# Intsights/PySubstringSearch

Measured on AMD Instinct MI355X. Metric: queries/sec (batched) + index-build GB/s on 512MB chunk, 1/2/4/8 GPU, higher is better.
Workload: dtype u64

## Files before the change

### pysubstringsearch_amd/csrc/msd_sort.hip

```cpp
#include "msd_sort.h"

#include <algorithm>
#include <type_traits>
#include <vector>

#include "prims.h"
#include "scan.h"
#include "text_keys.h"

namespace pss {

constexpr int MSD_D = 10;
constexpr u32 MSD_BINS = 1u << MSD_D;
constexpr int MSD_BLOCK = 512;
constexpr int MSD_WAVES = MSD_BLOCK / kWave;
constexpr int MSD_IPT = 16;
constexpr u32 MSD_TILE = MSD_BLOCK * MSD_IPT;
constexpr u32 MSD_WIN = 6144;
#ifndef PSS_LS_WINDOW
#define PSS_LS_WINDOW 8
#endif
constexpr u32 MSD_TILE_CAP = 8184 - PSS_LS_WINDOW;
constexpr u32 MSD_MAX_BUCKET = 4088;
constexpr int MSD_TAG_BITS = MSD_D + 1;
constexpr u32 MSD_TAG_SPAN = 1u << MSD_TAG_BITS;
constexpr int MSD_RAW_TAG_BITS = 6;
constexpr u32 MSD_RAW_TAG_SPAN = 1u << MSD_RAW_TAG_BITS;
constexpr u32 MSD_G1_RANGES = 1024;
constexpr u32 MSD_G2_RANGE = 16 * MSD_TILE;

struct MsdRange {
    u32 seg, start, end;
};

struct MsdTile2 {
    u32 start, count, d_last;
};

struct MsdArgs {
    const u8 *codes;
    int code_bits, key_chars, plus_one, key_drop;
    u32 n;
    int key_bits;
    int idx_bits;
    u32 tiles_per_range1, num_ranges1;
    u32 *T;
    u32 *J1;
    u32 *J;
    MsdRange *ranges2;
    u32 *seg_first;
    u32 *counters;
    const u64 *dense;
    const u64 *in;
    u64 *out;
    int lsd;
    u32 *T2;
    const u32 *Jb;
    const struct MsdTile2 *tiles2;
    u32 *status;
    const u8 *raw;
    const u8 *lut;
    u8 *codes_out;
    u32 *bad;
};

__device__ __forceinline__ void keep_load(u64 &v) { asm volatile("" : "+v"(v)); }
__device__ __forceinline__ void keep_load(uint4 &v) { asm volatile("" : "+v"(v.x), "+v"(v.y), "+v"(v.z), "+v"(v.w)); }

__device__ __forceinline__ void lds_barrier()
{
    asm volatile("s_waitcnt lgkmcnt(0)\n\ts_barrier" ::: "memory");
}


template <bool FROM_TEXT>
__device__ __forceinline__ void msd_load_tile(const MsdArgs &a, u32 base, u32 valid, u64 (&elem)[MSD_IPT], u32 (&dig)[MSD_IPT],
                                              int shift2)
{
    const u32 tid = threadIdx.x;
    if (FROM_TEXT) {
        const u32 i0 = base + tid * MSD_IPT;
        u64 key[MSD_IPT] = {};
        if (i0 < a.n) text_keys16(a.codes, i0, a.code_bits, a.key_chars, a.plus_one, a.key_drop, a.n, key);
        const int rest_bits = a.key_bits - MSD_D;
        const u64 rest_mask = (1ull << rest_bits) - 1ull;
#pragma unroll
        for (int r = 0; r < MSD_IPT; ++r) {
            dig[r] = (u32)(key[r] >> rest_bits) & (MSD_BINS - 1u);
            elem[r] = ((key[r] & rest_mask) << a.idx_bits) | (u64)(i0 + r);
        }
    } else {
#pragma unroll
        for (int r = 0; r < MSD_IPT; ++r) {
            const u32 p = r * MSD_BLOCK + tid;
            elem[r] = p < valid ? a.in[base + p] : 0ull;
            dig[r] = (u32)(elem[r] >> shift2) & (MSD_BINS - 1u);
        }
    }
}

template <bool FROM_TEXT>
__device__ __forceinline__ bool msd_valid(u32 base, u32 valid, int r, u32 n)
{
    const u32 tid = threadIdx.x;
    (void)base;
    (void)n;
    return FROM_TEXT ? (tid * MSD_IPT + r < valid) : (r * MSD_BLOCK + tid < valid);
}

template <bool FROM_TEXT>
__global__ __launch_bounds__(MSD_BLOCK) void msd_hist_kernel(MsdArgs a)
{
    __shared__ u32 hist[MSD_BINS];
    __shared__ u32 histb[FROM_TEXT ? MSD_BINS : 1];
    const u32 tid = threadIdx.x, r = blockIdx.x;
    u32 e0, e1;
    if (FROM_TEXT) {
        if (r >= a.num_ranges1) return;
        e0 = r * a.tiles_per_range1 * MSD_TILE;
        const u64 end = (u64)(r + 1) * a.tiles_per_range1 * MSD_TILE;
        e1 = end < a.n ? (u32)end : a.n;
    } else {
        if (r >= a.counters[0]) return;
        e0 = a.ranges2[r].start;
        e1 = a.ranges2[r].end;
    }
    for (u32 i = tid; i < MSD_BINS; i += MSD_BLOCK) {
        hist[i] = 0;
        if (FROM_TEXT) histb[i] = 0;
    }
    __syncthreads();
    const int shift2 = a.idx_bits + a.key_bits - 2 * MSD_D;
    if (FROM_TEXT) {
        const int b = a.code_bits;
        const int top = a.lsd ? 2 * MSD_D : MSD_D;
        const int m = (top + b - 1) / b;
        const u32 wmask = (m * b >= 32) ? ~0u : ((1u << (m * b)) - 1u);
        const int down = m * b - top;
        uint4 nlo = make_uint4(0, 0, 0, 0), nhi = nlo;
        if (e0 + tid * MSD_IPT < e1) {
            const uint4 *p = reinterpret_cast<const uint4 *>(a.codes + e0 + tid * MSD_IPT);
// ... 412 lines not shown
            if (lp[k] != 0xffffffffu) lp[k] = (lp[k] & 0xffffu) + (u32)s_start[lp[k] >> 22];
#pragma unroll
        for (int h = 0; h < MSD_PIECES2; ++h) {
            if (h * MSD_TILE >= valid) break;
            if (h) __syncthreads();
#pragma unroll
            for (int k = 0; k < IPT; ++k) {
                const u32 q = lp[k] - h * MSD_TILE;
                if (q < MSD_TILE) exch[q] = elem[k];
            }
            if (FROM_TEXT && h == MSD_PIECES2 - 1 && (u64)base + MSD_TILE2 < e1) load_ahead(base + MSD_TILE2);
            lds_barrier();
#pragma unroll
            for (int k = 0; k < (int)(MSD_TILE / BLOCK); ++k) {
                const u32 q = k * BLOCK + tid, p = h * MSD_TILE + q;
                if (p < valid) {
                    u64 e = exch[q];
                    u32 d;
                    if (FROM_TEXT) {
                        d = (u32)(e >> 14) & (MSD_BINS - 1u);
                        e = ((e >> 24) << a.idx_bits) | (u64)(base + ((u32)e & (MSD_TILE2 - 1u)));
                    } else {
                        d = (u32)(e >> shift2) & (MSD_BINS - 1u);
                        e = (e & low_mask2) | ((u64)(hist[d] >> 16) << shift2);
                    }
                    a.out[s_delta[d] + p] = e;
                }
            }
        }
    }
}

constexpr u32 LB_A = 1u << 30, LB_P = 2u << 30, LB_STATE = 3u << 30, LB_VALUE = LB_A - 1u;
constexpr int LB_WINDOW = 4;

struct LbAsk {
    u32 v[LB_WINDOW];
};
__device__ __forceinline__ void lb_ask(const u32 *status, u32 p, LbAsk &q)
{
#pragma unroll
    for (u32 w = 0; w < (u32)LB_WINDOW; ++w) {
        const u32 r = p > w ? p - 1 - w : 0u;
        q.v[w] = __hip_atomic_load(&status[(size_t)r * MSD_BINS + threadIdx.x], __ATOMIC_RELAXED, __HIP_MEMORY_SCOPE_AGENT);
    }
}
__device__ __forceinline__ void lb_begin(u32 *status, u32 t, u32 c, LbAsk &q)
{
    if (t == 0) return;
    __hip_atomic_store(&status[(size_t)t * MSD_BINS + threadIdx.x], LB_A | c, __ATOMIC_RELAXED, __HIP_MEMORY_SCOPE_AGENT);
    lb_ask(status, t, q);
}
__device__ __forceinline__ u32 lb_finish(u32 *status, u32 t, u32 c, u32 first, LbAsk &q)
{
    u32 off = first;
    if (t != 0) {
        u32 sum = 0, p = t;
        for (;;) {
            const u32 p0 = p;
            bool stop = false, done = false;
#pragma unroll
            for (u32 w = 0; w < (u32)LB_WINDOW; ++w) {
                if (!stop && w < p0) {
                    const u32 st = q.v[w] & LB_STATE;
                    if (st == 0) {
                        stop = true;
                    } else {
                        sum += q.v[w] & LB_VALUE;
                        --p;
                        if (st == LB_P) done = stop = true;
                    }
                }
            }
            if (done || p == 0) break;
            lb_ask(status, p, q);
        }
        off = sum;
    }
    __hip_atomic_store(&status[(size_t)t * MSD_BINS + threadIdx.x], LB_P | (off + c), __ATOMIC_RELAXED, __HIP_MEMORY_SCOPE_AGENT);
    return off;
}


__global__ __launch_bounds__(MSD_BINS) void msd_tiles2_kernel(const u32 *J1, MsdTile2 *tiles, u32 *counters)
{
    __shared__ u32 scr[MSD_BINS / kWave + 1];
    const u32 d = threadIdx.x;
    const u32 s = J1[d], e = J1[d + 1];
    const u32 nr = (e - s + MSD_TILE2 - 1) / MSD_TILE2;
    u32 total = 0, D = 0;
    const u32 first = block_excl_sum<MSD_BINS / kWave>(nr, scr, &total);
    const u32 dn = block_excl_sum<MSD_BINS / kWave>(nr ? 1u : 0u, scr, &D);
    if (d == 0) counters[0] = total + (MSD_BINS - D);
    if (nr == 0) {
        const u32 dd = D + (d - dn);
        tiles[total + (d - dn)] = MsdTile2{s, 0u, dd | 0x80000000u};
    }
    for (u32 k = 0; k < nr; ++k) {
        const u32 ts = s + k * MSD_TILE2;
        tiles[first + k] = MsdTile2{ts, min(MSD_TILE2, e - ts), dn | (k + 1 == nr ? 0x80000000u : 0u)};
    }
}

__global__ __launch_bounds__(1024) void msd_scatter_lb_kernel(MsdArgs a)
{
    constexpr int BLOCK = 1024;
    constexpr int IPT = MSD_TILE2 / BLOCK;
    __shared__ __attribute__((aligned(16))) u64 exch[MSD_TILE];
    __shared__ u32 hist[MSD_BINS], s_delta[MSD_BINS];
    __shared__ u16 s_start[MSD_BINS];
    __shared__ u32 scr[BLOCK / kWave + 1];
    __shared__ u32 s_ticket;
    const u32 tid = threadIdx.x;
    const u32 nt = a.counters[0];
    const int shift2 = a.idx_bits + a.key_bits - 2 * MSD_D;
    const u64 low_mask2 = (1ull << shift2) - 1ull;
    hist[tid] = 0;
    __syncthreads();
    for (;;) {
        if (tid == 0) s_ticket = atomicAdd(&a.counters[8], 1u);
        __syncthreads();
        const u32 t = s_ticket;
        if (t >= nt) break;
        const MsdTile2 td = a.tiles2[t];
        const u32 base = td.start, valid = td.count;
        u64 elem[IPT];
        u32 lp[IPT];
#pragma unroll
        for (int k = 0; k < IPT; ++k) {
            const u32 p = k * BLOCK + tid;
            elem[k] = p < valid ? a.in[base + p] : 0ull;
        }
#pragma unroll
        for (int k = 0; k < IPT; ++k) {
            const u32 p = k * BLOCK + tid;
            const u32 d = (u32)(elem[k] >> shift2) & (MSD_BINS - 1u);
            lp[k] = p < valid ? (atomicAdd(&hist[d], 1u) | (d << 22)) : 0xffffffffu;
        }
        __syncthreads();
        const u32 c = hist[tid];
        LbAsk ask;
        lb_begin(a.status, t, c, ask);
        const u32 ex = block_excl_sum<BLOCK / kWave>(c, scr, nullptr);
        s_start[tid] = (u16)ex;
        hist[tid] = 0;
        __syncthreads();
        const u64 tag = (u64)(td.d_last & (MSD_RAW_TAG_SPAN - 1u)) << shift2;
#pragma unroll
        for (int k = 0; k < IPT; ++k)
            if (lp[k] != 0xffffffffu) lp[k] = (lp[k] & 0xffffu) + (u32)s_start[lp[k] >> 22];
#pragma unroll
        for (int h = 0; h < MSD_PIECES2; ++h) {
            if (h && h * MSD_TILE >= valid) break;
            if (h) __syncthreads();
#pragma unroll
            for (int k = 0; k < IPT; ++k) {
                const u32 q = lp[k] - h * MSD_TILE;
                if (q < MSD_TILE) exch[q] = elem[k];
            }
            if (h == 0) {
                if (t == 0 && tid == 0) a.J[0] = 0;
                const u32 off = lb_finish(a.status, t, c, a.Jb[tid], ask);
                if (td.d_last >> 31) a.J[(size_t)tid * MSD_BINS + (td.d_last & (MSD_BINS - 1u)) + 1u] = off + c;
                s_delta[tid] = off - ex;
            }
            __syncthreads();
#pragma unroll
            for (int k = 0; k < (int)(MSD_TILE / BLOCK); ++k) {
                const u32 q = k * BLOCK + tid, p = h * MSD_TILE + q;
                if (p < valid) {
                    const u64 e = exch[q];
                    const u32 d = (u32)(e >> shift2) & (MSD_BINS - 1u);
                    a.out[s_delta[d] + p] = (e & low_mask2) | tag;
                }
            }
        }
    }
}


struct InNonEmpty {
    const u32 *J;
    __device__ u64 operator()(u64 j) const { return J[j + 1] > J[j] ? 1u : 0u; }
};

__global__ __launch_bounds__(256) void msd_compact_kernel(const u32 *J, u32 nb, const u64 *rank, u32 *cstart, u32 *counters, u32 *cj)
{
    u32 mx = 0;
    for (u32 j = blockIdx.x * blockDim.x + threadIdx.x; j < nb; j += gridDim.x * blockDim.x) {
        const u32 s = J[j], e = J[j + 1];
        if (e > s) {
            cstart[rank[j]] = s;
            if (cj) cj[rank[j]] = j;
            mx = max(mx, e - s);
        }
    }
    mx = wave_incl_max(mx);
    if (lane_id() == kWave - 1 && mx) atomicMax(&counters[1], mx);
}

struct TilePlan {
    u32 win, cap;
    const u32 *cj;
};
__device__ __forceinline__ bool msd_tile_head(const u32 *cstart, u32 ne, u32 n, u32 k, TilePlan tp)
{
    if (tp.cj) {
        if (k == 0 || (tp.cj[k] >> MSD_RAW_TAG_BITS) != (tp.cj[k - 1] >> MSD_RAW_TAG_BITS)) return true;
    } else if ((k & (MSD_TAG_SPAN - 1u)) == 0) {
        return true;
    }
    const u32 w = cstart[k] / tp.win;
    if (cstart[k - 1] / tp.win != w) return true;
    if (k + 1 < ne && cstart[k + 1] / tp.win == w) return false;
    u32 lo = 0, hi = k;
    const u32 ws = w * tp.win;
    while (lo < hi) {
        const u32 mid = (lo + hi) >> 1;
        if (cstart[mid] < ws) lo = mid + 1; else hi = mid;
    }
    const u32 end = k + 1 < ne ? cstart[k + 1] : n;
    return end - cstart[lo] > tp.cap;
}

struct InTileHead {
    const u32 *cstart;
    u32 ne, n;
    TilePlan tp;
    __device__ u64 operator()(u64 k) const { return msd_tile_head(cstart, ne, n, (u32)k, tp) ? 1u : 0u; }
};

struct InTileHeadDev {
    const u32 *cstart;
    const u64 *nep;
    u32 n;
    TilePlan tp;
    __device__ u64 operator()(u64 k) const
    {
        const u32 ne = (u32)*nep;
        return (k < ne && msd_tile_head(cstart, ne, n, (u32)k, tp)) ? 1u : 0u;
    }
};
__global__ __launch_bounds__(256) void msd_tiles_dev_kernel(const u32 *cstart, const u64 *nep, u32 n, const u64 *rank, const u64 *total,
                                                              u32 *tile_first, TilePlan tp)
{
    const u32 ne = (u32)*nep;
    if (blockIdx.x == 0 && threadIdx.x == 0) tile_first[*total] = ne;
    for (u32 k = blockIdx.x * blockDim.x + threadIdx.x; k < ne; k += gridDim.x * blockDim.x) {
        if (msd_tile_head(cstart, ne, n, k, tp)) tile_first[rank[k]] = k;
    }
}

__global__ __launch_bounds__(256) void msd_tiles_kernel(const u32 *cstart, u32 ne, u32 n, const u64 *rank, const u64 *total,
                                                          u32 *tile_first, TilePlan tp)
{
    if (blockIdx.x == 0 && threadIdx.x == 0) tile_first[*total] = ne;
    for (u32 k = blockIdx.x * blockDim.x + threadIdx.x; k < ne; k += gridDim.x * blockDim.x) {
        if (msd_tile_head(cstart, ne, n, k, tp)) tile_first[rank[k]] = k;
    }
// ... 533 lines not shown
            u32 ties = 0;
            ls_rows<LS_GROUP>(rows, [&](auto full, int g) __attribute__((always_inline)) {
                u64 cur[LS_GROUP], prv[LS_GROUP], nxt[LS_GROUP];
#pragma unroll
                for (int j = 0; j < LS_GROUP; ++j) {
                    const int o = (g + j) * MSD_BLOCK;
                    cur[j] = my[o];
                    prv[j] = o == 0 ? exch[tid - (tid != 0 ? 1u : 0u)] : my[o - 1];
                    nxt[j] = my[o + 1];
                }
#pragma unroll
                for (int j = 0; j < LS_GROUP; ++j) {
                    keep_load(cur[j]);
                    keep_load(prv[j]);
                    keep_load(nxt[j]);
                }
#pragma unroll
                for (int j = 0; j < LS_GROUP; ++j) {
                    const int o = (g + j) * MSD_BLOCK;
                    bool tie = (prv[j] ^ cur[j]) < same;
                    if (o == 0) tie = tie && tid != 0;
                    const bool tie_next = (nxt[j] ^ cur[j]) < same && (decltype(full)::value || o + tid + 1u < count);
                    if (decltype(full)::value || o + tid < count) {
                        out[o] = ((u32)cur[j] & imask) | (tie ? flag : 0u);
                        ties |= ((tie || tie_next) ? 1u << (g + j) : 0u) | (tie ? 0x10000u << (g + j) : 0u);
                    }
                }
            });
            if (em != nullptr) {
                u32 *const s_count = &scr[MSD_WAVES + 3];
                for (u32 m = ties & 0xffffu; m != 0; m &= m - 1u) {
                    const u32 r = (u32)__builtin_ctz(m);
                    const u32 p = r * MSD_BLOCK + tid;
                    const u32 slot = e0 + atomicAdd(s_count, 1u);
                    em->st_pos[slot] = e0 + p;
                    em->st_idx[slot] = ((u32)exch[p] & imask) | ((ties >> (16u + r)) << 31);
                }
            }
        }
        prev_t = t;
        prev_ok = !failed;
        if (!more) break;
        t += stride;
        cur = nxt;
        nxt = t + stride < nt ? tiles[t + stride] : MsdTile{0, 0, 0, 0};
    }
    if (em) {
        lds_barrier();
        if (tid == 0 && prev_ok) em->blk_cnt[prev_t] = scr[MSD_WAVES + 3];
    }
}

#include "ss_sort_impl.h"


static size_t msd_max_tiles(uint32_t n)
{
    return (size_t)n / (SS_WIN / 2) + ((size_t)MSD_BINS * MSD_BINS) / MSD_RAW_TAG_SPAN + 8;
}

static size_t msd_max_tiles2(uint32_t n) { return (size_t)n / MSD_TILE2 + MSD_BINS + 8; }

static bool msd_use_lsd(uint32_t n)
{
    const char *e = knob("PSS_MSD_LSD");
    return !(e && atoi(e) == 0) && n < (1u << 30);
}

size_t msd_workspace_bytes(uint32_t n)
{
    const size_t max_ranges2 = (size_t)n / MSD_G2_RANGE + MSD_BINS + 8;
    const size_t nbk = (size_t)MSD_BINS * MSD_BINS;
    return max_ranges2 * MSD_BINS * 4
           + (MSD_BINS + 8) * 4
           + (nbk + 8) * 4
           + max_ranges2 * sizeof(MsdRange) + (MSD_BINS + 8) * 4 + 64
           + (nbk + 8) * 8
           + (nbk + 8) * 4
           + (msd_max_tiles(n) + 32) * 8
           + (msd_max_tiles(n) + 32) * 16
           + (msd_max_tiles(n) + 32) * sizeof(MsdTile)
           + (SC_MAX_BLOCKS + 8) * 8 + 8192
           + (size_t)MSD_BINS * MSD_G1_RANGES * 4 + (MSD_BINS + 8) * 4
           + msd_max_tiles2(n) * (sizeof(MsdTile2) + (size_t)MSD_BINS * 4)
           + (nbk + 8) * 4 + 4096;
}

int msd_max_key_bits(uint32_t n)
{
    int ib = 1;
    while ((1ull << ib) < (u64)n) ++ib;
    const int after2 = 64 + MSD_D - (msd_use_lsd(n) ? MSD_RAW_TAG_BITS : MSD_TAG_BITS) - ib + MSD_D;
    return std::min(after2, 64 + MSD_D - ib);
}

int msd_suffix_sort(DeviceCtx *ctx, const TextKeys *text, uint32_t n, int key_bits, uint64_t *A[2], uint32_t *sa_out,
                    void *work, uint32_t *h_small, bool profile, MsdStats *stats, bool *accepted, MsdActive *active,
                    const MsdFront *front)
{
    *accepted = false;
    hipStream_t s = ctx->stream;
    int ib = 1;
    while ((1ull << ib) < (u64)n) ++ib;
    if (key_bits < 2 * MSD_D + 1 || key_bits > msd_max_key_bits(n) || n < 2) {
        set_error("msd_suffix_sort: key of %d bits does not fit (n = %u)", key_bits, n);
        return PSS_EINVAL;
    }
    const size_t max_ranges2 = (size_t)n / MSD_G2_RANGE + MSD_BINS + 8;
    const size_t nbk = (size_t)MSD_BINS * MSD_BINS;
    u8 *w = static_cast<u8 *>(work);
    size_t o = 0;
    auto carve = [&](size_t bytes) { u8 *p = w + o; o = round_up(o + bytes, 256); return p; };
    u32 *T = reinterpret_cast<u32 *>(carve(max_ranges2 * MSD_BINS * 4));
    u32 *J1 = reinterpret_cast<u32 *>(carve((MSD_BINS + 8) * 4));
    u32 *J = reinterpret_cast<u32 *>(carve((nbk + 8) * 4));
    MsdRange *ranges2 = reinterpret_cast<MsdRange *>(carve(max_ranges2 * sizeof(MsdRange)));
    u32 *seg_first = reinterpret_cast<u32 *>(carve((MSD_BINS + 8) * 4));
    u32 *counters = reinterpret_cast<u32 *>(carve(64));
    u64 *ranks = reinterpret_cast<u64 *>(carve((nbk + 8) * 8));
    u32 *cstart = reinterpret_cast<u32 *>(carve((nbk + 8) * 4));
    const size_t max_tiles = msd_max_tiles(n);
    MsdTile *tiles_all = reinterpret_cast<MsdTile *>(carve((max_tiles + 16) * sizeof(MsdTile)));
    u32 *tile_first = reinterpret_cast<u32 *>(carve((max_tiles + 16) * 8));
    u32 *blk_cnt = reinterpret_cast<u32 *>(carve((max_tiles + 8) * 4));
    u64 *dst_off = reinterpret_cast<u64 *>(carve((max_tiles + 8) * 8));
    u64 *partial = reinterpret_cast<u64 *>(carve((SC_MAX_BLOCKS + 8) * 8));
    u64 *d_total = partial + SC_MAX_BLOCKS;
    const bool lsd = msd_use_lsd(n);
    const size_t max_tiles2 = msd_max_tiles2(n);
    u32 *T2 = nullptr, *Jb = nullptr, *status = nullptr, *cj = nullptr;
    MsdTile2 *tiles2 = nullptr;
    if (lsd) {
        T2 = reinterpret_cast<u32 *>(carve((size_t)MSD_BINS * MSD_G1_RANGES * 4));
        Jb = reinterpret_cast<u32 *>(carve((MSD_BINS + 8) * 4));
        tiles2 = reinterpret_cast<MsdTile2 *>(carve(max_tiles2 * sizeof(MsdTile2)));
        status = reinterpret_cast<u32 *>(carve(max_tiles2 * MSD_BINS * 4));
        cj = reinterpret_cast<u32 *>(carve((nbk + 8) * 4));
    }

    MsdArgs a;
    memset(&a, 0, sizeof a);
    a.codes = text->codes;
    a.code_bits = text->code_bits;
    a.key_chars = text->key_chars;
    a.plus_one = text->plus_one;
    a.key_drop = text->drop;
    a.n = n;
    a.key_bits = key_bits;
    a.idx_bits = ib;
    const u32 num_tiles = (u32)(((u64)n + MSD_TILE - 1) / MSD_TILE);
    a.tiles_per_range1 = (num_tiles + MSD_G1_RANGES - 1) / MSD_G1_RANGES;
    a.num_ranges1 = (num_tiles + a.tiles_per_range1 - 1) / a.tiles_per_range1;
    a.T = T;
    a.J1 = J1;
    a.J = J;
    a.ranges2 = ranges2;
    a.seg_first = seg_first;
    a.counters = counters;
    a.lsd = lsd ? 1 : 0;
    a.T2 = T2;
    a.Jb = Jb;
    a.tiles2 = tiles2;
    a.status = status;

    hipEvent_t ev[8] = {};
    int nev = 0;
    struct EvGuard {
        hipEvent_t *e;
        int *n;
        ~EvGuard()
        {
            for (int i = 0; i < *n; ++i) (void)hipEventDestroy(e[i]);
        }
    } guard{ev, &nev};
    auto mark = [&]() -> int {
        if (profile && nev < 8) {
            PSS_HIP(hipEventCreate(&ev[nev]));
            PSS_HIP(hipEventRecord(ev[nev], s));
            ++nev;
        }
        return PSS_OK;
    };

    PSS_HIP(hipMemsetAsync(counters, 0, 64, s));
    a.out = A[0];
    if (front) {
        a.raw = front->raw;
        a.lut = front->lut;
        a.codes_out = const_cast<u8 *>(text->codes);
        a.bad = front->bad;
        hipLaunchKernelGGL(msd_hist_raw_kernel, dim3(a.num_ranges1), dim3(MSD_BLOCK), 0, s, a);
    } else {
        hipLaunchKernelGGL(msd_hist_kernel<true>, dim3(a.num_ranges1), dim3(MSD_BLOCK), 0, s, a);
    }
    static_assert(MSD_G1_RANGES <= 1024, "msd_offsets1_kernel takes four ranges per thread");
    hipLaunchKernelGGL(msd_offsets1_kernel, dim3(MSD_BINS), dim3(256), 0, s, T, a.num_ranges1, seg_first);
    hipLaunchKernelGGL(msd_offsets1b_kernel, dim3(1), dim3(MSD_BINS), 0, s, (const u32 *)seg_first, J1, n);
    if (lsd) {
        hipLaunchKernelGGL(msd_offsets1_kernel, dim3(MSD_BINS), dim3(256), 0, s, T2, a.num_ranges1, seg_first);
        hipLaunchKernelGGL(msd_offsets1b_kernel, dim3(1), dim3(MSD_BINS), 0, s, (const u32 *)seg_first, Jb, n);
        PSS_HIP(hipMemsetAsync(status, 0, max_tiles2 * MSD_BINS * 4, s));
    }
    PSS_TRY(mark());
    const bool wide = lsd || !(knob("PSS_MSD_SCATTER") && atoi(knob("PSS_MSD_SCATTER")) == 1);
    if (lsd) hipLaunchKernelGGL((msd_scatter2_kernel<true, 1024, true>), dim3(a.num_ranges1), dim3(1024), 0, s, a);
    else if (wide) hipLaunchKernelGGL((msd_scatter2_kernel<true, 1024>), dim3(a.num_ranges1), dim3(1024), 0, s, a);
    else hipLaunchKernelGGL(msd_scatter_kernel<true>, dim3(a.num_ranges1), dim3(MSD_BLOCK), 0, s, a);
    PSS_TRY(mark());
    a.in = A[0];
    a.out = A[1];
    if (lsd) {
        hipLaunchKernelGGL(msd_tiles2_kernel, dim3(1), dim3(MSD_BINS), 0, s, (const u32 *)J1, tiles2, counters);
        PSS_TRY(mark());
        const u32 grid2 = std::min<u32>((u32)max_tiles2, (u32)ctx->num_cus);
        hipLaunchKernelGGL(msd_scatter_lb_kernel, dim3(grid2), dim3(1024), 0, s, a);
        PSS_TRY(mark());
    } else {
        hipLaunchKernelGGL(msd_ranges_kernel, dim3(1), dim3(MSD_BINS), 0, s, J1, ranges2, seg_first, counters);
        a.dense = ranks;
        hipLaunchKernelGGL(msd_hist_kernel<false>, dim3((u32)max_ranges2), dim3(MSD_BLOCK), 0, s, a);
        hipLaunchKernelGGL(msd_offsets_kernel, dim3(MSD_BINS), dim3(MSD_BINS), 0, s, T, (const u32 *)seg_first, (const u32 *)J1, J,
                           0u, n, MSD_BINS);
    }
    PSS_TRY(device_excl_scan(ctx, InNonEmpty{J}, nbk, partial, d_total, ranks));
    hipLaunchKernelGGL(msd_compact_kernel, dim3(1024), dim3(256), 0, s, J, (u32)nbk, ranks, cstart, counters, cj);
    const int rem_bits = key_bits - 2 * MSD_D;
    MsdEmit em{};
    const int fused = active != nullptr;
    if (fused) em = MsdEmit{active->st_pos, active->st_idx, blk_cnt};
    const bool one_trip = lsd && !knob("PSS_MSD_SLOW_LOCAL");
    u64 *d_total2 = d_total + 1;
    u32 *const fail_list_dev = tile_first + max_tiles + 16;
    if (one_trip) {
        const TilePlan tpd{MSD_WIN, MSD_TILE_CAP, cj};
        PSS_TRY(device_excl_scan(ctx, InTileHeadDev{cstart, d_total, n, tpd}, nbk, partial, d_total2, ranks));
        hipLaunchKernelGGL(msd_tiles_dev_kernel, dim3(1024), dim3(256), 0, s, cstart, (const u64 *)d_total, n, ranks, (const u64 *)d_total2,
                           tile_first, tpd);
        hipLaunchKernelGGL(msd_tile_desc_kernel, dim3((u32)((max_tiles + 255) / 256)), dim3(256), 0, s, cstart, tile_first, 0u, 0u, n,
                           tiles_all, (const u32 *)cj, (const u64 *)d_total2, (const u64 *)d_total);
        PSS_TRY(mark());
        hipLaunchKernelGGL(msd_local_fast_kernel, dim3(2u * (u32)ctx->num_cus), dim3(MSD_BLOCK), 0, s, A[1], (const MsdTile *)tiles_all, 0u,
                           rem_bits, ib, sa_out, fail_list_dev, counters + 4, fused, em, (const u64 *)d_total2, (const u32 *)counters,
                           front ? (const u32 *)front->bad : (const u32 *)nullptr);
        PSS_TRY(mark());
        PSS_HIP(hipMemcpyAsync(h_small + 8, d_total2, 8, hipMemcpyDeviceToHost, s));
        PSS_HIP(hipMemcpyAsync(h_small + 10, counters + 4, 4, hipMemcpyDeviceToHost, s));
    }
    PSS_HIP(hipMemcpyAsync(h_small, d_total, 8, hipMemcpyDeviceToHost, s));
    PSS_HIP(hipMemcpyAsync(h_small + 2, counters, 16, hipMemcpyDeviceToHost, s));
    if (front) PSS_HIP(hipMemcpyAsync(h_small + 6, front->bad, 4, hipMemcpyDeviceToHost, s));
    PSS_HIP(hipStreamSynchronize(s));
    const u32 ne = h_small[0];
    const u32 maxb = h_small[3];
    if (stats) {
        stats->buckets = ne;
        stats->max_bucket = maxb;
        stats->bad_symbol = front ? h_small[6] : 0u;
    }
    if (front && h_small[6]) return PSS_OK;
    if (maxb > MSD_MAX_BUCKET) return PSS_OK;
    if (!lsd) {
        PSS_TRY(mark());
        if (wide) hipLaunchKernelGGL((msd_scatter2_kernel<false, 1024>), dim3((u32)max_ranges2), dim3(1024), 0, s, a);
        else hipLaunchKernelGGL(msd_scatter_kernel<false>, dim3((u32)max_ranges2), dim3(MSD_BLOCK), 0, s, a);
        PSS_TRY(mark());
    }
    const auto local_sort = msd_local_sort_kernel;
    const auto local_fast = msd_local_fast_kernel;
    u32 nt = 0;
    u32 *fail_list = fail_list_dev;
    if (one_trip) {
        nt = h_small[8];
        if ((size_t)nt > max_tiles) {
            set_error("msd_suffix_sort: %u tiles planned, tables hold %zu (internal error)", nt, max_tiles);
            return PSS_EDEVICE;
        }
        const u32 nfail = h_small[10];
        if (stats) stats->slow_tiles = nfail;
        if (nfail)
            hipLaunchKernelGGL(local_sort, dim3(nfail), dim3(MSD_BLOCK), 0, s, A[1], (const MsdTile *)tiles_all, rem_bits,
                               ib, sa_out, (const u32 *)fail_list, fused, em);
    } else {
    const TilePlan tp{MSD_WIN, MSD_TILE_CAP, cj};
    PSS_TRY(device_excl_scan(ctx, InTileHead{cstart, ne, n, tp}, ne, partial, d_total, ranks));
    hipLaunchKernelGGL(msd_tiles_kernel, dim3(1024), dim3(256), 0, s, cstart, ne, n, ranks, (const u64 *)d_total, tile_first, tp);
    PSS_HIP(hipMemcpyAsync(h_small, d_total, 8, hipMemcpyDeviceToHost, s));
    PSS_HIP(hipStreamSynchronize(s));
    nt = h_small[0];
    if ((size_t)nt > max_tiles) {
        set_error("msd_suffix_sort: %u tiles planned, tables hold %zu (internal error)", nt, max_tiles);
        return PSS_EDEVICE;
    }
    PSS_TRY(mark());
    fail_list = tile_first + nt + 8;
    hipLaunchKernelGGL(msd_tile_desc_kernel, dim3((nt + 255) / 256), dim3(256), 0, s, cstart, tile_first, nt, ne, n, tiles_all,
                       (const u32 *)cj, (const u64 *)nullptr, (const u64 *)nullptr);
    if (knob("PSS_MSD_SLOW_LOCAL")) {
// ... 332 lines not shown
```

### pysubstringsearch_amd/csrc/common.cpp

```cpp
#include "common.h"
#include "knobs.h"

#include <atomic>
#include <cstring>
#include <cstdio>
#include <cstdlib>
#include <algorithm>
#include <cerrno>
#include <unistd.h>

#include <mutex>
#include <vector>

namespace pss {

static thread_local std::string g_err;

void set_error(const char *fmt, ...)
{
    char buf[1024];
    va_list ap;
    va_start(ap, fmt);
    vsnprintf(buf, sizeof buf, fmt, ap);
    va_end(ap);
// ... 292 lines not shown
{
    int count = 0;
    hipError_t e = hipGetDeviceCount(&count);
    if (e != hipSuccess || count <= 0) {
        (void)hipGetLastError();
        set_error("no usable HIP device (%s); libpss has no CPU fallback",
                  e != hipSuccess ? hipGetErrorString(e) : "device count is 0");
        return PSS_EDEVICE;
    }
    if (device < 0 || device >= count || device >= kMaxDevices) {
        set_error("device %d out of range (have %d)", device, count);
        return PSS_EINVAL;
    }
    PSS_HIP(hipSetDevice(device));
    std::lock_guard<std::mutex> lk(g_ctx_mu);
    DeviceCtx &c = table[device];
    if (c.device < 0) PSS_TRY(init_ctx(c, device));
    *out = &c;
    return PSS_OK;
}

int get_helper_ctx(DeviceCtx *parent, DeviceCtx **out)
{
    if (!parent->helper) {
        DeviceCtx *h = new DeviceCtx();
        const int rc = init_ctx(*h, parent->device);
        if (rc != PSS_OK) {
            delete h;
            return rc;
        }
        parent->helper = h;
    }
    *out = parent->helper;
    return PSS_OK;
}

int get_ctx(int device, DeviceCtx **out) { return get_ctx_of(g_ctx, device, out); }
int get_build_ctx(int device, DeviceCtx **out) { return get_ctx_of(g_bctx, device, out); }

int DeviceCtx::ensure_resident()
{
    if (resident.arena) return PSS_OK;
    PSS_HIP(hipStreamCreateWithFlags(&resident.stream, hipStreamNonBlocking));
    PSS_HIP(hipHostMalloc(&resident.arena, kPinnedBytes, hipHostMallocCoherent | hipHostMallocMapped));
    PSS_HIP(hipHostGetDevicePointer(&resident.arena_dev, resident.arena, 0));
    memset(resident.arena, 0, kPinnedBytes);
    return PSS_OK;
}

void DeviceCtx::Resident::post(const uint8_t *q, uint32_t plen)
{
    ResidentMailbox *mb = reinterpret_cast<ResidentMailbox *>(static_cast<uint8_t *>(arena) + kResidentMailboxOff);
    if (plen != kResidentStop) {
        if (plen <= sizeof mb->post.bytes) {
            memcpy(mb->post.bytes, q, plen);
        } else {
            memcpy(mb->query, q, plen);
            memset(mb->query + plen, 0, 32);
        }
    }
    mb->post.plen = plen;
    ++seq;
    __atomic_store_n(&mb->post.seq_b, seq, __ATOMIC_RELEASE);
    __atomic_store_n(&mb->post.seq_a, seq, __ATOMIC_RELEASE);
}

void DeviceCtx::stop_resident()
{
    if (!resident.running) return;
    resident.post(nullptr, kResidentStop);
    (void)hipStreamSynchronize(resident.stream);
    resident.running = false;
}

const KnobDef kKnobs[] = {
    {"PSS_KEY_CHARS", "0 (chosen)", "1|2|3|5|8|12|16", "builder: force the symbols packed into the initial sort key"},
    {"PSS_KEY_DROP", "-1 (chosen)", "0|1|3|7", "builder: force the low bits of the last key symbol that are left out"},
    {"PSS_NO_SAMPLE", "unset", "1", "builder: size the initial key from symbol counts even for large texts (no sizing sample)"},
    {"PSS_NO_TIES_PASS", "unset", "1", "builder: plain 8-byte-key LSD passes and key comparison in the rerank (no tie flags)"},
    {"PSS_MODE", "chosen", "dense|sparse|text", "builder: how ties are resolved -- doubling over an inverse suffix array, sparse (hash), text rounds"},
    {"PSS_TEXT_ROUNDS", "5", "0|1|2|3", "builder: text rounds at most before the rank rounds"},
    {"PSS_MSD", "-1 (screened)", "0|1|1", "initial sort: never / whenever the key fits the hybrid MSD radix sort (msd_sort.hip)"},
    {"PSS_MSD_LSD", "1", "0|1", "MSD sort: 0 = digits in MSD order with a second histogram pass (rounds 2-5); else LSD order, second pass by look-back"},
    {"PSS_MSD_KEY_CAP", "48", "", "MSD sort: largest key width tried (bits; the element format bounds it further)"},
    {"PSS_MSD_PARTIAL_SYMBOL", "unset", "1", "MSD sort: fill the element with the high bits of one more symbol than fits whole (fewer ties; measured slower on lines)"},
    {"PSS_MSD_NO_FUSE", "unset", "1", "MSD sort: ties flagged in the suffix array instead of emitted from the local sort"},
    {"PSS_MSD_NO_FINISH", "unset", "1", "MSD sort: small tie groups go to the rounds instead of being finished by one more text key after the local sort"},
    {"PSS_MSD_SLOW_LOCAL", "unset", "1", "MSD sort: the general (ballot LSD) local-sort kernel for every tile"},
    {"PSS_MSD_SCATTER", "unset", "1", "MSD sort in MSD order: the 8192-element partition kernels of round 2"},
    {"PSS_SS", "-1 (n >= 2^24, MSD declined)", "0|1", "initial sort: never / whenever the text has the size for it the sample sort over 16-byte elements"},
    {"PSS_SS_SEG", "1", "0", "sample sort: 0 = every tile merge-sorted as one array instead of bucket by bucket"},
    {"PSS_SS_WINDOW_PLAN", "unset", "1", "sample sort: tiles by the window rule of the MSD sort instead of the greedy plan"},
    {"PSS_SS_DEBUG", "unset", "", "sample sort: print where a bucket beyond a tile came from (diagnostic)"},
    {"PSS_NO_PLAN_CACHE", "unset", "1", "builder: forget between chunks which initial sort and alphabet the previous chunk took"},
    {"PSS_NO_PLAN_FRONT", "unset", "1", "builder: remember the sort but not the alphabet (separate alphabet and recode passes)"},
    {"PSS_RLE", "-1 (runs average >= 8 bytes)", "0|1|1", "builder: never / always the run-length path (rle_build.hip)"},
    {"PSS_RLE_SORT", "unset", "1", "run-length path: expansion by the stable radix sort instead of the matrix walk"},
    {"PSS_PERIOD", "-1 (when the text repeats one word)", "0", "builder: 0 = never the closed form for a text that repeats one word"},
    {"PSS_ANCHOR", "-1 (texts of >= 2^20 bytes)", "0|1|1", "builder: never / whenever ties outlive the text rounds the anchor round (anchor_impl.h)"},
    {"PSS_ANCHOR_OMEGA", "0 (as wide as the common prefix allows)", "9|12|17|33", "anchor round: force the window of the minimizers"},
    {"PSS_ANCHOR_MIN_OMEGA", "11", "3|7|9", "anchor round: narrowest window it accepts by itself"},
    {"PSS_ANCHOR_SIDE", "-1 (>= 2^24 bytes, sampled ties show copies)", "0|1", "anchor round: never / always sort the anchors beside the text round (second stream)"},
    {"PSS_ANCHOR_SIDE_PCT", "8", "", "anchor round: share of sampled tied pairs that must be copies for the side line"},
    {"PSS_ANCHOR_CAP_DIV", "5", "3|4", "anchor round: declines above n / this many anchors"},
    {"PSS_NO_PROBE", "unset", "1", "builder: always a text round before the anchor round (no sampling of the ties)"},
    {"PSS_PROBE_SKIP_PCT", "50", "0|20|90", "builder: no text rounds when more than this share of the sampled tied pairs are repeats"},
    {"PSS_NO_MID_TIER", "unset", "1", "rounds: groups above 512 members all take the chained radix sorts"},
    {"PSS_NO_MID_MERGE", "unset", "1", "rounds: groups of 513 .. 4096 members with a crowded bin take the chained sorts (no LDS merge sort)"},
    {"PSS_BIG_MERGE", "-1 (by the average size of the large groups)", "0|1|2", "rounds: groups above 4096 members through the segmented merge sort (2: in text rounds only)"},
    {"PSS_NO_BIG_MERGE", "unset", "", "rounds: overrides PSS_BIG_MERGE"},
    {"PSS_COUNT_SORT", "unset", "1", "rank rounds: groups ranked by counting instead of the merge sort"},
    {"PSS_PERIODIC", "1", "0", "rank rounds: 0 = no periodic keys for the large groups"},
    {"PSS_TIMING", "unset", "", "builder / Writer: per-round and per-stage trace on stderr"},
    {"PSS_DEVICES", "all visible", "0|0,0|0,0,0|all", "devices of Reader(path) / Writer(path) without a device argument: all | comma-separated ordinals"},
    {"PSS_DEVICE", "unset", "", "default device of a process (launchers' LOCAL_RANK etc. are honoured the same way)"},
    {"PSS_IO_THREADS", "8 .. 16 by core count", "2|5", "file path: threads of the I/O pool"},
    {"PSS_INGEST_BLOCK", "32 MiB", "16|40|300", "Writer: size of the direct reads of add_entries_from_file_lines"},
    {"PSS_INGEST_MIN_ROOM", "1 MiB", "1|20", "Writer: room a chunk must have left for one direct read"},
    {"PSS_WRITER_MMAP", "tmpfs: 1, else 0", "0|1", "Writer: records through a shared mapping (1) or pwrite (0)"},
    {"PSS_WRITER_MMAP_MIN", "1 MiB", "16", "Writer: smallest record that goes through the mapping"},
    {"PSS_WRITER_HOST_BUDGET", "8 GiB", "", "multi-device Writer: host text of the chunks in flight (one chunk always goes through)"},
    {"PSS_STRIPES", "8", "", "striped container format 2: stripe files of a Writer"},
    {"PSS_EXPERIMENT_NO_FILE", "unset", "", "measurement only: the record thread copies without writing the file"},
    {"PSS_RESULT_ORDER", "text", "sa", "Reader: 'sa' = the reference's order inside a chunk (suffix-array order of every entry's first hit)"},
    {"PSS_READER_HBM_BUDGET", "whatever hipMalloc grants minus 2 GiB", "", "Reader: suffix arrays beyond this many bytes of HBM stay in pinned host memory"},
    {"PSS_READER_AUTO_RESIDENCY", "1", "", "Reader: 0 = the residency manager never moves a suffix array by itself"},
    {"PSS_NO_KEY_SAMPLES", "unset", "", "Reader: no key-sample table"},
    {"PSS_SAMPLE_SHIFT", "11", "", "Reader: one key sample per 2^shift suffixes"},
    {"PSS_LINE_BLOCK_SHIFT", "8", "6|7|9|10", "Reader: the line index behind entry ids keeps one newline rank per 2^shift bytes of text (6 .. 10)"},
    {"PSS_NO_SMALL_PATH", "unset", "1", "search: no fused single-query kernels"},
    {"PSS_NO_BLOCK_PATH", "unset", "1", "search: small batches one wave per pair instead of one workgroup"},
    {"PSS_NO_SEARCH_STAGE", "unset", "1", "search: no pinned staging of queries and results"},
    {"PSS_WAVE_SEARCH", "unset", "1", "search: interval kernel one wave per pair at every batch size"},
    {"PSS_NO_GROUP_SEARCH", "unset", "1", "search: never 16 lanes per pair"},
    {"PSS_NO_MID_PIPELINE", "unset", "1", "search: always the general multi-kernel pipeline"},
    {"PSS_PINNED_POOL_BYTES", "40 GiB", "", "search: pinned host memory the result pool keeps between batches"},
    {"PSS_NO_PINNED_RESULTS", "unset", "1", "search: large results into pageable memory"},
    {"PSS_LANE_SEARCH_MIN", "8192", "1|100000", "search: pairs from which one lane per pair searches"},
    {"PSS_ICASE_SEED_LETTERS", "5", "1|2|3|4|5|6", "case-insensitive search: ASCII letters of a pattern's seed at most (2^letters spellings probed per pattern and chunk)"},
    {"PSS_SEARCH_EVENTS", "unset", "", "single-query path: HIP events around the fused kernel (fills ms_device; ~4 us per query)"},
    {"PSS_RESIDENT_IDLE_US", "1000", "", "low-latency mode: the resident kernel leaves after this long without a query"},
    {"PSS_RESIDENT_LIFE_US", "50000", "", "low-latency mode: ... and after this long in any case"},
    {"PSS_TRACE_RESIDENT", "unset", "", "libpss_trace.so only: print the resident kernel's phase stamps"},
    {"PSS_RCCL_LIB", "librccl.so of the process", "", "gather inside the C ABI: the RCCL library to load"},
    {"PSS_RCCL_TIMEOUT_MS", "60000", "", "gather inside the C ABI: bound of every wait for the peers"},
};
const int kNumKnobs = (int)(sizeof(kKnobs) / sizeof(kKnobs[0]));

const char *knob(const char *name)
{
    for (int i = 0; i < kNumKnobs; ++i)
        if (strcmp(kKnobs[i].name, name) == 0) return getenv(name);
    static std::atomic<bool> said{false};
    if (!said.exchange(true)) fprintf(stderr, "[pss] %s is not in the switch registry (knobs.h): treated as unset\n", name);
    return nullptr;
}

uint64_t workspace_bytes(int device)
{
    if (device < 0 || device >= kMaxDevices) return 0;
    std::lock_guard<std::mutex> lk(g_ctx_mu);
    uint64_t total = 0;
    for (DeviceCtx *table : {g_ctx, g_bctx}) {
        DeviceCtx &c = table[device];
        if (c.device < 0) continue;
        for (auto &s : c.slot) total += s.cap;
// ... 32 lines not shown
```

Before: 72.25.

## Prefetch next scatter tile ticket during last piece and specialize full tiles

The decoupled-lookback scatter kernel now issues the atomic ticket for its next tile early, during the last rows of the current tile's final scatter piece, using inline asm with a deferred vmcnt wait. It then loads the tile descriptor through scalar loads and publishes it in shared memory, so the atomic and descriptor latency overlap with the scatter stores. The tile body is also templated on whether the tile is full, which removes bounds checks in the common case. The costs are dependence on hand-written GCN asm and waitcnt counting that must stay correct, and extra code size from the two template instantiations.

Result: no change. 72.66, median of 6 (+0.6%).

```diff
diff --git a/pysubstringsearch_amd/csrc/msd_sort.hip b/pysubstringsearch_amd/csrc/msd_sort.hip
--- a/pysubstringsearch_amd/csrc/msd_sort.hip
+++ b/pysubstringsearch_amd/csrc/msd_sort.hip
@@ -28,6 +28,11 @@
 constexpr u32 MSD_RAW_TAG_SPAN = 1u << MSD_RAW_TAG_BITS;
 constexpr u32 MSD_G1_RANGES = 1024;
 constexpr u32 MSD_G2_RANGE = 16 * MSD_TILE;
+
+#ifndef PSS_LB_TICKET_ROWS
+#define PSS_LB_TICKET_ROWS 8
+#endif
+static_assert(PSS_LB_TICKET_ROWS >= 0 && PSS_LB_TICKET_ROWS <= 8, "the ticket is asked for inside the tile's last piece");
 
 struct MsdRange {
     u32 seg, start, end;
@@ -655,40 +660,54 @@
     }
 }
 
-__global__ __launch_bounds__(1024) void msd_scatter_lb_kernel(MsdArgs a)
+__device__ __forceinline__ void lb_ticket_ask(u32 *counter, u32 &tk)
+{
+    asm volatile("global_atomic_add %0, %1, %0, off sc0" : "+v"(tk) : "v"(counter) : "memory");
+}
+template <int BEHIND>
+__device__ __forceinline__ void lb_ticket_wait(u32 &tk)
+{
+    asm volatile("s_waitcnt vmcnt(%1)" : "+v"(tk) : "n"(BEHIND) : "memory");
+}
+__device__ __forceinline__ void lb_ticket_publish(const MsdTile2 *tiles, u32 nt, u32 tk, u32 *s_next)
+{
+    const u32 t = __builtin_amdgcn_readfirstlane(tk);
+    u64 lo = 0;
+    u32 hi = 0;
+    if (t < nt) {
+        const MsdTile2 *p = tiles + t;
+        asm volatile("s_load_dwordx2 %0, %2, 0x0\n\ts_load_dword %1, %2, 0x8\n\ts_waitcnt lgkmcnt(0)"
+                     : "=&s"(lo), "=&s"(hi)
+                     : "s"(p)
+                     : "memory");
+    }
+    *reinterpret_cast<uint4 *>(s_next) = make_uint4(t, (u32)lo, (u32)(lo >> 32), hi);
+}
+
+template <bool FULL>
+__device__ __forceinline__ void lb_tile(const MsdArgs &a, u32 nt, u32 t, const MsdTile2 td, int shift2, u64 low_mask2, u64 *exch,
+                                        u32 *hist, u32 *s_delta, u16 *s_start, u32 *scr, u32 *s_next)
 {
     constexpr int BLOCK = 1024;
     constexpr int IPT = MSD_TILE2 / BLOCK;
-    __shared__ __attribute__((aligned(16))) u64 exch[MSD_TILE];
-    __shared__ u32 hist[MSD_BINS], s_delta[MSD_BINS];
-    __shared__ u16 s_start[MSD_BINS];
-    __shared__ u32 scr[BLOCK / kWave + 1];
-    __shared__ u32 s_ticket;
+    constexpr int ROWS = MSD_TILE / BLOCK;
+    constexpr int ASK = FULL ? PSS_LB_TICKET_ROWS : 0;
     const u32 tid = threadIdx.x;
-    const u32 nt = a.counters[0];
-    const int shift2 = a.idx_bits + a.key_bits - 2 * MSD_D;
-    const u64 low_mask2 = (1ull << shift2) - 1ull;
-    hist[tid] = 0;
-    __syncthreads();
-    for (;;) {
-        if (tid == 0) s_ticket = atomicAdd(&a.counters[8], 1u);
-        __syncthreads();
-        const u32 t = s_ticket;
-        if (t >= nt) break;
-        const MsdTile2 td = a.tiles2[t];
-        const u32 base = td.start, valid = td.count;
+    {
+        const u32 base = td.start, valid = FULL ? MSD_TILE2 : td.count;
+        u32 tk = 1u;
         u64 elem[IPT];
         u32 lp[IPT];
 #pragma unroll
         for (int k = 0; k < IPT; ++k) {
             const u32 p = k * BLOCK + tid;
-            elem[k] = p < valid ? a.in[base + p] : 0ull;
+            elem[k] = (FULL || p < valid) ? a.in[base + p] : 0ull;
         }
 #pragma unroll
         for (int k = 0; k < IPT; ++k) {
             const u32 p = k * BLOCK + tid;
             const u32 d = (u32)(elem[k] >> shift2) & (MSD_BINS - 1u);
-            lp[k] = p < valid ? (atomicAdd(&hist[d], 1u) | (d << 22)) : 0xffffffffu;
+            lp[k] = (FULL || p < valid) ? (atomicAdd(&hist[d], 1u) | (d << 22)) : 0xffffffffu;
         }
         __syncthreads();
         const u32 c = hist[tid];
@@ -701,10 +720,10 @@
         const u64 tag = (u64)(td.d_last & (MSD_RAW_TAG_SPAN - 1u)) << shift2;
 #pragma unroll
         for (int k = 0; k < IPT; ++k)
-            if (lp[k] != 0xffffffffu) lp[k] = (lp[k] & 0xffffu) + (u32)s_start[lp[k] >> 22];
+            if (FULL || lp[k] != 0xffffffffu) lp[k] = (lp[k] & 0xffffu) + (u32)s_start[lp[k] >> 22];
 #pragma unroll
         for (int h = 0; h < MSD_PIECES2; ++h) {
-            if (h && h * MSD_TILE >= valid) break;
+            if (!FULL && h && h * MSD_TILE >= valid) break;
             if (h) __syncthreads();
 #pragma unroll
             for (int k = 0; k < IPT; ++k) {
@@ -719,15 +738,52 @@
             }
             __syncthreads();
 #pragma unroll
-            for (int k = 0; k < (int)(MSD_TILE / BLOCK); ++k) {
+            for (int k = 0; k < ROWS; ++k) {
+                if (ASK > 0 && h == MSD_PIECES2 - 1 && k == ROWS - ASK && tid == 0) lb_ticket_ask(&a.counters[8], tk);
                 const u32 q = k * BLOCK + tid, p = h * MSD_TILE + q;
-                if (p < valid) {
+                if (FULL || p < valid) {
                     const u64 e = exch[q];
                     const u32 d = (u32)(e >> shift2) & (MSD_BINS - 1u);
                     a.out[s_delta[d] + p] = (e & low_mask2) | tag;
                 }
             }
         }
+        if (tid == 0) {
+            if (ASK == 0) lb_ticket_ask(&a.counters[8], tk);
+            lb_ticket_wait<ASK>(tk);
+            lb_ticket_publish(a.tiles2, nt, tk, s_next);
+        }
+    }
+}
+
+__global__ __launch_bounds__(1024) void msd_scatter_lb_kernel(MsdArgs a)
+{
+    constexpr int BLOCK = 1024;
+    __shared__ __attribute__((aligned(16))) u64 exch[MSD_TILE];
+    __shared__ u32 hist[MSD_BINS], s_delta[MSD_BINS];
+    __shared__ u16 s_start[MSD_BINS];
+    __shared__ u32 scr[BLOCK / kWave + 1];
+    __shared__ __attribute__((aligned(16))) u32 s_next[4];
+    const u32 tid = threadIdx.x;
+    const u32 nt = a.counters[0];
+    const int shift2 = a.idx_bits + a.key_bits - 2 * MSD_D;
+    const u64 low_mask2 = (1ull << shift2) - 1ull;
+    hist[tid] = 0;
+    if (tid == 0) {
+        u32 tk = 1u;
+        lb_ticket_ask(&a.counters[8], tk);
+        lb_ticket_wait<0>(tk);
+        lb_ticket_publish(a.tiles2, nt, tk, s_next);
+    }
+    for (;;) {
+        __syncthreads();
+        const uint4 nx = *reinterpret_cast<const uint4 *>(s_next);
+        const u32 t = __builtin_amdgcn_readfirstlane(nx.x);
+        if (t >= nt) break;
+        const MsdTile2 td{(u32)__builtin_amdgcn_readfirstlane(nx.y), (u32)__builtin_amdgcn_readfirstlane(nx.z),
+                          (u32)__builtin_amdgcn_readfirstlane(nx.w)};
+        if (td.count == MSD_TILE2) lb_tile<true>(a, nt, t, td, shift2, low_mask2, exch, hist, s_delta, s_start, scr, s_next);
+        else lb_tile<false>(a, nt, t, td, shift2, low_mask2, exch, hist, s_delta, s_start, scr, s_next);
     }
 }
 
```

## Prefetch next tile in look-back scatter and derive tile descriptors from per-digit regions

Applied to the files above, without the earlier changes.

The persistent look-back scatter kernel now grabs its next ticket and loads the next tile's elements while the current tile's second half is still being written, overlapping global loads with output writes. Tile descriptors are no longer materialized per tile. The kernel keeps per-digit region tables (first tile, start, size) in LDS and finds a tile's digit with two wave ballots. A knob to cap the persistent grid size is added for experiments. The change costs extra LDS and register pressure and makes the ordering logic harder to follow.

Result: no change. 72.90 before, 73.71 after, median of 5 (+1.1%).

```diff
diff --git a/pysubstringsearch_amd/csrc/common.cpp b/pysubstringsearch_amd/csrc/common.cpp
--- a/pysubstringsearch_amd/csrc/common.cpp
+++ b/pysubstringsearch_amd/csrc/common.cpp
@@ -398,6 +398,7 @@
     {"PSS_TEXT_ROUNDS", "5", "0|1|2|3", "builder: text rounds at most before the rank rounds"},
     {"PSS_MSD", "-1 (screened)", "0|1|1", "initial sort: never / whenever the key fits the hybrid MSD radix sort (msd_sort.hip)"},
     {"PSS_MSD_LSD", "1", "0|1", "MSD sort: 0 = digits in MSD order with a second histogram pass (rounds 2-5); else LSD order, second pass by look-back"},
+    {"PSS_MSD_LB_GRID", "unset (one per CU)", "1|2|3", "MSD sort in LSD order: persistent workgroups of the look-back pass at most (1: one workgroup takes every tile in turn)"},
     {"PSS_MSD_KEY_CAP", "48", "", "MSD sort: largest key width tried (bits; the element format bounds it further)"},
     {"PSS_MSD_PARTIAL_SYMBOL", "unset", "1", "MSD sort: fill the element with the high bits of one more symbol than fits whole (fewer ties; measured slower on lines)"},
     {"PSS_MSD_NO_FUSE", "unset", "1", "MSD sort: ties flagged in the suffix array instead of emitted from the local sort"},
diff --git a/pysubstringsearch_amd/csrc/msd_sort.hip b/pysubstringsearch_amd/csrc/msd_sort.hip
--- a/pysubstringsearch_amd/csrc/msd_sort.hip
+++ b/pysubstringsearch_amd/csrc/msd_sort.hip
@@ -36,6 +36,7 @@
 struct MsdTile2 {
     u32 start, count, d_last;
 };
+constexpr u32 MSD_REGIONS2_WORDS = 3 * MSD_BINS;
 
 struct MsdArgs {
     const u8 *codes;
@@ -56,7 +57,7 @@
     int lsd;
     u32 *T2;
     const u32 *Jb;
-    const struct MsdTile2 *tiles2;
+    const u32 *regions2;
     u32 *status;
     const u8 *raw;
     const u8 *lut;
@@ -635,7 +636,7 @@
 }
 
 
-__global__ __launch_bounds__(MSD_BINS) void msd_tiles2_kernel(const u32 *J1, MsdTile2 *tiles, u32 *counters)
+__global__ __launch_bounds__(MSD_BINS) void msd_tiles2_kernel(const u32 *J1, u32 *regions, u32 *counters)
 {
     __shared__ u32 scr[MSD_BINS / kWave + 1];
     const u32 d = threadIdx.x;
@@ -645,14 +646,19 @@
     const u32 first = block_excl_sum<MSD_BINS / kWave>(nr, scr, &total);
     const u32 dn = block_excl_sum<MSD_BINS / kWave>(nr ? 1u : 0u, scr, &D);
     if (d == 0) counters[0] = total + (MSD_BINS - D);
-    if (nr == 0) {
-        const u32 dd = D + (d - dn);
-        tiles[total + (d - dn)] = MsdTile2{s, 0u, dd | 0x80000000u};
-    }
-    for (u32 k = 0; k < nr; ++k) {
-        const u32 ts = s + k * MSD_TILE2;
-        tiles[first + k] = MsdTile2{ts, min(MSD_TILE2, e - ts), dn | (k + 1 == nr ? 0x80000000u : 0u)};
-    }
+    const u32 dd = nr ? dn : D + (d - dn);
+    regions[dd] = nr ? first : total + (d - dn);
+    regions[MSD_BINS + dd] = s;
+    regions[2 * MSD_BINS + dd] = e - s;
+}
+
+__device__ __forceinline__ MsdTile2 msd_tile2_of(const u32 *r_first, const u32 *r_start, const u32 *r_size, u32 t)
+{
+    const u32 lane = lane_id();
+    const u32 blk = (u32)__popcll(__ballot(r_first[16u * lane] <= t)) - 1u;
+    const u32 dn = 16u * blk + (u32)__popcll(__ballot(lane < 16u && r_first[16u * blk + (lane & 15u)] <= t)) - 1u;
+    const u32 at = (t - r_first[dn]) * MSD_TILE2, left = r_size[dn] - at;
+    return MsdTile2{r_start[dn] + at, min(MSD_TILE2, left), dn | (left <= MSD_TILE2 ? 0x80000000u : 0u)};
 }
 
 __global__ __launch_bounds__(1024) void msd_scatter_lb_kernel(MsdArgs a)
@@ -663,27 +669,52 @@
     __shared__ u32 hist[MSD_BINS], s_delta[MSD_BINS];
     __shared__ u16 s_start[MSD_BINS];
     __shared__ u32 scr[BLOCK / kWave + 1];
-    __shared__ u32 s_ticket;
+    __shared__ u32 r_first[MSD_BINS], r_start[MSD_BINS], r_size[MSD_BINS];
+    __shared__ u32 s_next[4];
     const u32 tid = threadIdx.x;
     const u32 nt = a.counters[0];
     const int shift2 = a.idx_bits + a.key_bits - 2 * MSD_D;
     const u64 low_mask2 = (1ull << shift2) - 1ull;
     hist[tid] = 0;
+    r_first[tid] = a.regions2[tid];
+    r_start[tid] = a.regions2[MSD_BINS + tid];
+    r_size[tid] = a.regions2[2 * MSD_BINS + tid];
     __syncthreads();
-    for (;;) {
-        if (tid == 0) s_ticket = atomicAdd(&a.counters[8], 1u);
-        __syncthreads();
-        const u32 t = s_ticket;
-        if (t >= nt) break;
-        const MsdTile2 td = a.tiles2[t];
-        const u32 base = td.start, valid = td.count;
-        u64 elem[IPT];
-        u32 lp[IPT];
+    u32 ticket = 0;
+    auto ask_ticket = [&]() __attribute__((always_inline)) {
+        if (tid == 0) ticket = atomicInc(&a.counters[8], 0xffffffffu);
+    };
+    auto publish_next = [&]() __attribute__((always_inline)) {
+        if (tid < (u32)kWave) {
+            const u32 t = __builtin_amdgcn_readfirstlane(ticket);
+            MsdTile2 td{0u, 0u, 0u};
+            if (t < nt) td = msd_tile2_of(r_first, r_start, r_size, t);
+            if (tid == 0) {
+                s_next[0] = t;
+                s_next[1] = td.start;
+                s_next[2] = td.count;
+                s_next[3] = td.d_last;
+            }
+        }
+    };
+    u64 elem[IPT];
+    auto load_tile = [&](u32 base, u32 valid) __attribute__((always_inline)) {
 #pragma unroll
         for (int k = 0; k < IPT; ++k) {
             const u32 p = k * BLOCK + tid;
             elem[k] = p < valid ? a.in[base + p] : 0ull;
         }
+    };
+    ask_ticket();
+    publish_next();
+    __syncthreads();
+    u32 t = __builtin_amdgcn_readfirstlane(s_next[0]);
+    u32 valid = __builtin_amdgcn_readfirstlane(s_next[2]), d_last = __builtin_amdgcn_readfirstlane(s_next[3]);
+    load_tile(__builtin_amdgcn_readfirstlane(s_next[1]), valid);
+    while (t < nt) {
+        u32 lp[IPT];
+#pragma unroll
+        for (int k = 0; k < IPT; ++k) keep_load(elem[k]);
 #pragma unroll
         for (int k = 0; k < IPT; ++k) {
             const u32 p = k * BLOCK + tid;
@@ -698,26 +729,19 @@
         s_start[tid] = (u16)ex;
         hist[tid] = 0;
         __syncthreads();
-        const u64 tag = (u64)(td.d_last & (MSD_RAW_TAG_SPAN - 1u)) << shift2;
+        const u64 tag = (u64)(d_last & (MSD_RAW_TAG_SPAN - 1u)) << shift2;
 #pragma unroll
         for (int k = 0; k < IPT; ++k)
             if (lp[k] != 0xffffffffu) lp[k] = (lp[k] & 0xffffu) + (u32)s_start[lp[k] >> 22];
-#pragma unroll
-        for (int h = 0; h < MSD_PIECES2; ++h) {
-            if (h && h * MSD_TILE >= valid) break;
-            if (h) __syncthreads();
+        const bool two = valid > MSD_TILE;
+        auto stage = [&](u32 h) __attribute__((always_inline)) {
 #pragma unroll
             for (int k = 0; k < IPT; ++k) {
                 const u32 q = lp[k] - h * MSD_TILE;
                 if (q < MSD_TILE) exch[q] = elem[k];
             }
-            if (h == 0) {
-                if (t == 0 && tid == 0) a.J[0] = 0;
-                const u32 off = lb_finish(a.status, t, c, a.Jb[tid], ask);
-                if (td.d_last >> 31) a.J[(size_t)tid * MSD_BINS + (td.d_last & (MSD_BINS - 1u)) + 1u] = off + c;
-                s_delta[tid] = off - ex;
-            }
-            __syncthreads();
+        };
+        auto write_out = [&](u32 h) __attribute__((always_inline)) {
 #pragma unroll
             for (int k = 0; k < (int)(MSD_TILE / BLOCK); ++k) {
                 const u32 q = k * BLOCK + tid, p = h * MSD_TILE + q;
@@ -727,7 +751,33 @@
                     a.out[s_delta[d] + p] = (e & low_mask2) | tag;
                 }
             }
-        }
+        };
+        stage(0);
+        {
+            if (t == 0 && tid == 0) a.J[0] = 0;
+            const u32 off = lb_finish(a.status, t, c, a.Jb[tid], ask);
+            if (d_last >> 31) a.J[(size_t)tid * MSD_BINS + (d_last & (MSD_BINS - 1u)) + 1u] = off + c;
+            s_delta[tid] = off - ex;
+        }
+        ask_ticket();
+        if (two) {
+            __syncthreads();
+            write_out(0);
+            publish_next();
+            __syncthreads();
+            stage(1);
+        } else {
+            publish_next();
+            __syncthreads();
+        }
+        const u32 nx_t = __builtin_amdgcn_readfirstlane(s_next[0]), nx_valid = __builtin_amdgcn_readfirstlane(s_next[2]);
+        const u32 nx_d_last = __builtin_amdgcn_readfirstlane(s_next[3]);
+        load_tile(__builtin_amdgcn_readfirstlane(s_next[1]), nx_valid);
+        lds_barrier();
+        write_out(two ? 1u : 0u);
+        t = nx_t;
+        valid = nx_valid;
+        d_last = nx_d_last;
     }
 }
 
@@ -1427,7 +1477,7 @@
            + (msd_max_tiles(n) + 32) * sizeof(MsdTile)
            + (SC_MAX_BLOCKS + 8) * 8 + 8192
            + (size_t)MSD_BINS * MSD_G1_RANGES * 4 + (MSD_BINS + 8) * 4
-           + msd_max_tiles2(n) * (sizeof(MsdTile2) + (size_t)MSD_BINS * 4)
+           + (MSD_REGIONS2_WORDS + 64) * 4 + msd_max_tiles2(n) * (size_t)MSD_BINS * 4
            + (nbk + 8) * 4 + 4096;
 }
 
@@ -1474,11 +1524,11 @@
     const bool lsd = msd_use_lsd(n);
     const size_t max_tiles2 = msd_max_tiles2(n);
     u32 *T2 = nullptr, *Jb = nullptr, *status = nullptr, *cj = nullptr;
-    MsdTile2 *tiles2 = nullptr;
+    u32 *regions2 = nullptr;
     if (lsd) {
         T2 = reinterpret_cast<u32 *>(carve((size_t)MSD_BINS * MSD_G1_RANGES * 4));
         Jb = reinterpret_cast<u32 *>(carve((MSD_BINS + 8) * 4));
-        tiles2 = reinterpret_cast<MsdTile2 *>(carve(max_tiles2 * sizeof(MsdTile2)));
+        regions2 = reinterpret_cast<u32 *>(carve(MSD_REGIONS2_WORDS * 4));
         status = reinterpret_cast<u32 *>(carve(max_tiles2 * MSD_BINS * 4));
         cj = reinterpret_cast<u32 *>(carve((nbk + 8) * 4));
     }
@@ -1505,7 +1555,7 @@
     a.lsd = lsd ? 1 : 0;
     a.T2 = T2;
     a.Jb = Jb;
-    a.tiles2 = tiles2;
+    a.regions2 = regions2;
     a.status = status;
 
     hipEvent_t ev[8] = {};
@@ -1555,9 +1605,11 @@
     a.in = A[0];
     a.out = A[1];
     if (lsd) {
-        hipLaunchKernelGGL(msd_tiles2_kernel, dim3(1), dim3(MSD_BINS), 0, s, (const u32 *)J1, tiles2, counters);
+        hipLaunchKernelGGL(msd_tiles2_kernel, dim3(1), dim3(MSD_BINS), 0, s, (const u32 *)J1, regions2, counters);
         PSS_TRY(mark());
-        const u32 grid2 = std::min<u32>((u32)max_tiles2, (u32)ctx->num_cus);
+        u32 grid2 = std::min<u32>((u32)max_tiles2, (u32)ctx->num_cus);
+        if (const char *e = knob("PSS_MSD_LB_GRID"))
+            if (atoi(e) > 0) grid2 = std::min<u32>(grid2, (u32)atoi(e));
         hipLaunchKernelGGL(msd_scatter_lb_kernel, dim3(grid2), dim3(1024), 0, s, a);
         PSS_TRY(mark());
     } else {
```
